# daviesthomas/cudaNeuralRender

Hardware: AMD Instinct MI355X
Metric: Mray-steps/s at 1024^2, plane_1.h5 (frames/s in config.fps) (higher is better)
Workload: dtype f32

## Files before the change

cudaneuralrender_amd/csrc/nr_mlp16.h:

```cpp
#pragma once
#include <type_traits>

#include "nr_device.h"
#include "nr_mlp16_asm.h"

#ifndef NR_MLP16_EXP
#define NR_MLP16_EXP 0
#endif

namespace nr {

typedef float f32x4 __attribute__((ext_vector_type(4)));

__device__ __forceinline__ uint32_t pl16(uint32_t a, uint32_t b, int half) {
    const auto r = __builtin_amdgcn_permlane16_swap(a, b, false, false);
    return half ? r[1] : r[0];
}
__device__ __forceinline__ uint32_t pl32(uint32_t a, uint32_t b, int half) {
    const auto r = __builtin_amdgcn_permlane32_swap(a, b, false, false);
    return half ? r[1] : r[0];
}

template <int NT>
__device__ __forceinline__ float tile_outputs(const float zt[4]) {
// ... 46 lines not shown
#pragma unroll
    for (int t = 0; t < NT; ++t)
#pragma unroll
        for (int i = 0; i < 8; ++i) a[t][i] = k[t][i];
}

template <int NT, int PART = 0, bool CL = false, int NH = 0, bool MK = false>
__device__ __forceinline__ float mlp16_fp32_nt(const float *__restrict__ s, int in0, int nh_rt, float fr, float x,
                                               float y, float z, uint32_t (*mk)[2] = nullptr) {
    const int nh = NH > 0 ? NH : nh_rt;
    auto relu = [](float v) { return CL ? __builtin_amdgcn_fmed3f(v, 0.0f, 1.0f) : fmaxf(v, 0.0f); };
    auto mark = [](uint32_t m, float act, int pos) { return (min(__float_as_uint(act), 1u) << pos) | m; };
    const int lane = lane_id(), g = lane >> 4;
    float a[NT][8];
    f32x4 c[NT][2];
    {
        const float w0 = s[PK_L0W + lane], w1 = s[PK_L0W + 64 + lane];
        uint32_t t0 = __float_as_uint(x), t1 = __float_as_uint(y), t2 = __float_as_uint(z);
        uint32_t t3 = __float_as_uint(in0 == 4 ? fr : 0.0f);
        auto r = __builtin_amdgcn_permlane32_swap(t0, t2, false, false);
        t0 = r[0]; t2 = r[1];
        r = __builtin_amdgcn_permlane32_swap(t1, t3, false, false);
        t1 = r[0]; t3 = r[1];
        r = __builtin_amdgcn_permlane16_swap(t0, t1, false, false);
        t0 = r[0]; t1 = r[1];
        r = __builtin_amdgcn_permlane16_swap(t2, t3, false, false);
        t2 = r[0]; t3 = r[1];
        const float bt[4] = {__uint_as_float(t0), __uint_as_float(t1), __uint_as_float(t2), __uint_as_float(t3)};
#pragma unroll
        for (int t = 0; t < NT; ++t) {
            c[t][0] = __builtin_amdgcn_mfma_f32_16x16x4f32(w0, bt[t], f32x4{0.0f, 0.0f, 0.0f, 0.0f}, 0, 0, 0);
            c[t][1] = __builtin_amdgcn_mfma_f32_16x16x4f32(w1, bt[t], f32x4{0.0f, 0.0f, 0.0f, 0.0f}, 0, 0, 0);
        }
        const float4 *bb = reinterpret_cast<const float4 *>(s + PK_L0B + g * 8);
        const float4 blo = bb[0], bhi = bb[1];
        const float bias[8] = {blo.x, blo.y, blo.z, blo.w, bhi.x, bhi.y, bhi.z, bhi.w};
        const float s0 = s[pk_final(nh) + 33];
#pragma unroll
        for (int t = 0; t < NT; ++t)
#pragma unroll
            for (int mt = 0; mt < 2; ++mt)
#pragma unroll
                for (int r = 0; r < 4; ++r) {
                    a[t][4 * mt + r] = relu(__builtin_fmaf(c[t][mt][r], s0, bias[4 * mt + r]));
                    if constexpr (MK) mk[t][0] = mark(mk[t][0], a[t][4 * mt + r], 4 * mt + r);
                }
    }
    constexpr bool STREAM = NT <= 2 && CL && NH == 7 && PART == 0;
    if constexpr (STREAM) f32_hidden7_stream<NT>(s, a);
    for (int jl = 0; jl < (STREAM ? 0 : nh); ++jl) {
        const float *L = s + PK_HID + jl * PK_HID_STRIDE;
        float4 wq[4];
#pragma unroll
        for (int q = 0; q < 4; ++q) wq[q] = reinterpret_cast<const float4 *>(L)[q * 64 + lane];
#pragma unroll
        for (int st = 0; st < 8; ++st) {
#pragma unroll
            for (int mt = 0; mt < 2; ++mt) {
                const int m = 2 * st + mt;
                const float4 wv = wq[m >> 2];
                const float w = (m & 3) == 0 ? wv.x : ((m & 3) == 1 ? wv.y : ((m & 3) == 2 ? wv.z : wv.w));
#pragma unroll
                for (int t = 0; t < NT; ++t)
                    c[t][mt] = __builtin_amdgcn_mfma_f32_16x16x4f32(
                        w, a[t][st], st == 0 ? f32x4{0.0f, 0.0f, 0.0f, 0.0f} : c[t][mt], 0, 0, 0);
            }
        }
        const float4 *bb = reinterpret_cast<const float4 *>(L + 1024 + g * 8);
        const float4 blo = bb[0], bhi = bb[1];
        const float bias[8] = {blo.x, blo.y, blo.z, blo.w, bhi.x, bhi.y, bhi.z, bhi.w};
#pragma unroll
        for (int t = 0; t < NT; ++t)
#pragma unroll
            for (int mt = 0; mt < 2; ++mt)
#pragma unroll
                for (int r = 0; r < 4; ++r) a[t][4 * mt + r] = relu(c[t][mt][r] + bias[4 * mt + r]);
        if constexpr (MK) {
            const int pos = 8 * ((jl + 1) & 3);
#pragma unroll
            for (int t = 0; t < NT; ++t)
#pragma unroll
                for (int k = 0; k < 8; ++k) {
                    if (jl + 1 < 4) mk[t][0] = mark(mk[t][0], a[t][k], pos + k);
                    else mk[t][1] = mark(mk[t][1], a[t][k], pos + k);
                }
        }
    }
    if constexpr (PART != 0) return a[0][0] + a[NT - 1][7];
    if constexpr (NT >= 3) {
        float b[4][8];
#pragma unroll
        for (int k = 0; k < 8; ++k) {
            uint32_t t0 = __float_as_uint(a[0][k]), t1 = __float_as_uint(a[1][k]);
            uint32_t t2 = __float_as_uint(a[2][k]), t3 = NT > 3 ? __float_as_uint(a[NT > 3 ? 3 : 0][k]) : 0u;
            auto r = __builtin_amdgcn_permlane32_swap(t0, t2, false, false);
            t0 = r[0]; t2 = r[1];
            r = __builtin_amdgcn_permlane32_swap(t1, t3, false, false);
            t1 = r[0]; t3 = r[1];
            r = __builtin_amdgcn_permlane16_swap(t0, t1, false, false);
            t0 = r[0]; t1 = r[1];
            r = __builtin_amdgcn_permlane16_swap(t2, t3, false, false);
            t2 = r[0]; t3 = r[1];
            b[0][k] = __uint_as_float(t0); b[1][k] = __uint_as_float(t1);
            b[2][k] = __uint_as_float(t2); b[3][k] = __uint_as_float(t3);
        }
        const float4 *wf4 = reinterpret_cast<const float4 *>(s + pk_final(nh));
        float acc = 0.0f;
#pragma unroll
        for (int q = 0; q < 8; ++q) {
            const float4 w = wf4[q];
            const int gg = q >> 1, k0 = 4 * (q & 1);
            acc = __builtin_fmaf(w.x, b[gg][k0 + 0], acc);
            acc = __builtin_fmaf(w.y, b[gg][k0 + 1], acc);
            acc = __builtin_fmaf(w.z, b[gg][k0 + 2], acc);
            acc = __builtin_fmaf(w.w, b[gg][k0 + 3], acc);
        }
        return acc + s[pk_final(nh) + 32];
    }
    const float *wf = s + pk_final(nh) + g * 8;
    const float bf = s[pk_final(nh) + 32];
    float w8[8];
#pragma unroll
    for (int k = 0; k < 8; ++k) w8[k] = wf[k];
    float zt[4] = {0.0f, 0.0f, 0.0f, 0.0f};
#pragma unroll
    for (int t = 0; t < NT; ++t) {
        float acc = 0.0f;
#pragma unroll
        for (int k = 0; k < 8; ++k) acc = __builtin_fmaf(w8[k], a[t][k], acc);
#pragma unroll
        for (int q = 1; q < 4; ++q) {
            float nacc = from_prev_group(acc, q);
#pragma unroll
            for (int k = 0; k < 8; ++k) nacc = __builtin_fmaf(w8[k], a[t][k], nacc);
            acc = (g == q) ? nacc : acc;
        }
        zt[t] = acc + bf;
    }
    return tile_outputs<NT>(zt);
}

__device__ __forceinline__ bool inputs_in_bound_f32(float x, float y, float z, float f) {
    const bool ok = __builtin_fabsf(x) <= F32_INPUT_BOUND && __builtin_fabsf(y) <= F32_INPUT_BOUND &&
                    __builtin_fabsf(z) <= F32_INPUT_BOUND && __builtin_fabsf(f) <= F32_INPUT_BOUND;
    return __ballot(!ok) == 0;
}

template <bool ST = false>
__device__ __forceinline__ float mlp16_fp32(const float *__restrict__ s, int in0, int nh, float fr, float x, float y,
                                            float z, uint32_t tmask, bool cl) {
    const int nt = 32 - __clz((int)tmask);
    if (cl) {
        if (nt >= 4) return mlp16_fp32_nt<4, 0, true>(s, in0, nh, fr, x, y, z);
        if (nt == 3) return mlp16_fp32_nt<3, 0, true>(s, in0, nh, fr, x, y, z);
        if (nt == 2) return mlp16_fp32_nt<2, 0, true>(s, in0, nh, fr, x, y, z);
        if (ST && NR_F32_STREAM && nh == 7) return mlp16_fp32_nt<1, 0, true, 7>(s, in0, nh, fr, x, y, z);
        if (nt == 2) return mlp16_fp32_nt<2, 0, true>(s, in0, nh, fr, x, y, z);
        return mlp16_fp32_nt<1, 0, true>(s, in0, nh, fr, x, y, z);
    }
    return mlp16_fp32_nt<4>(s, in0, nh, fr, x, y, z);
}
template <bool ST = false>
__device__ __forceinline__ float mlp16_fp32(const MlpArgs &M, const float *s, float fr, float x, float y, float z,
                                            uint32_t tmask) {
    return mlp16_fp32<ST>(s, M.in0, M.nh, fr, x, y, z, tmask, M.f32_clamp && inputs_in_bound_f32(x, y, z, fr));
}

__device__ __forceinline__ int prune_ks(unsigned long long kb, int l) { return 4 + (int)((kb >> (3 * l)) & 7ull); }

template <int NT>
__device__ __forceinline__ float mlp16_fp32_pruned_nt(const float *__restrict__ s, int in0, int nh, unsigned long long kb,
                                                      float fr, float x, float y, float z, uint32_t &flag) {
    auto relu = [](float v) { return __builtin_amdgcn_fmed3f(v, 0.0f, 1.0f); };
    const int lane = lane_id(), g = lane >> 4;
    f32x4 av[NT][2];
    f32x4 c[NT][2];
    uint32_t fl = 0;
    auto skipped = [&](int k) {
#pragma unroll
        for (int t = 0; t < NT; t += 2) fl |= __float_as_uint(av[t][k >> 2][k & 3]) | __float_as_uint(av[t + 1 < NT ? t + 1 : t][k >> 2][k & 3]);
    };
    {
        const float w0 = s[PK_L0W + lane], w1 = s[PK_L0W + 64 + lane];
        uint32_t t0 = __float_as_uint(x), t1 = __float_as_uint(y), t2 = __float_as_uint(z);
        uint32_t t3 = __float_as_uint(in0 == 4 ? fr : 0.0f);
        auto r = __builtin_amdgcn_permlane32_swap(t0, t2, false, false);
        t0 = r[0]; t2 = r[1];
        r = __builtin_amdgcn_permlane32_swap(t1, t3, false, false);
        t1 = r[0]; t3 = r[1];
        r = __builtin_amdgcn_permlane16_swap(t0, t1, false, false);
        t0 = r[0]; t1 = r[1];
        r = __builtin_amdgcn_permlane16_swap(t2, t3, false, false);
        t2 = r[0]; t3 = r[1];
        const float bt[4] = {__uint_as_float(t0), __uint_as_float(t1), __uint_as_float(t2), __uint_as_float(t3)};
#pragma unroll
        for (int t = 0; t < NT; ++t) {
            c[t][0] = __builtin_amdgcn_mfma_f32_16x16x4f32(w0, bt[t], f32x4{0.0f, 0.0f, 0.0f, 0.0f}, 0, 0, 0);
            c[t][1] = __builtin_amdgcn_mfma_f32_16x16x4f32(w1, bt[t], f32x4{0.0f, 0.0f, 0.0f, 0.0f}, 0, 0, 0);
        }
        const float4 *bb = reinterpret_cast<const float4 *>(s + PK_L0B + g * 8);
        const float4 blo = bb[0], bhi = bb[1];
        const float bias[8] = {blo.x, blo.y, blo.z, blo.w, bhi.x, bhi.y, bhi.z, bhi.w};
        const float s0 = s[pk_final(nh) + 33];
#pragma unroll
        for (int t = 0; t < NT; ++t)
#pragma unroll
            for (int mt = 0; mt < 2; ++mt)
#pragma unroll
                for (int r = 0; r < 4; ++r) av[t][mt][r] = relu(__builtin_fmaf(c[t][mt][r], s0, bias[4 * mt + r]));
    }
    for (int jl = 0; jl < nh; ++jl) {
        const int ks = prune_ks(kb, jl);
        const float *L = s + PK_HID + jl * PK_HID_STRIDE;
        float4 wq[2];
#pragma unroll
        for (int q = 0; q < 2; ++q) wq[q] = reinterpret_cast<const float4 *>(L)[q * 64 + lane];
#pragma unroll
        for (int st = 0; st < 8; ++st) {
            if (st < 4 || st < ks) {
                float2 w2 = {0.0f, 0.0f};
                if (st >= 4) w2 = reinterpret_cast<const float2 *>(L)[((st >> 1) * 64 + lane) * 2 + (st & 1)];
#pragma unroll
                for (int mt = 0; mt < 2; ++mt) {
                    const int m = 2 * st + mt;
                    const float4 wv = wq[st < 4 ? m >> 2 : 0];
                    const float w4 = (m & 3) == 0 ? wv.x : ((m & 3) == 1 ? wv.y : ((m & 3) == 2 ? wv.z : wv.w));
                    const float w = st < 4 ? w4 : (mt ? w2.y : w2.x);
#pragma unroll
                    for (int t = 0; t < NT; ++t)
                        c[t][mt] = __builtin_amdgcn_mfma_f32_16x16x4f32(
                            w, av[t][st >> 2][st & 3], st == 0 ? f32x4{0.0f, 0.0f, 0.0f, 0.0f} : c[t][mt], 0, 0, 0);
                }
            }
        }
        if (ks < 8) {
#pragma unroll
            for (int k = 4; k < 8; ++k)
                if (k >= ks) skipped(k);
        }
        const float4 *bb = reinterpret_cast<const float4 *>(L + 1024 + g * 8);
        const float4 blo = bb[0], bhi = bb[1];
        const float bias[8] = {blo.x, blo.y, blo.z, blo.w, bhi.x, bhi.y, bhi.z, bhi.w};
#pragma unroll
        for (int t = 0; t < NT; ++t)
#pragma unroll
            for (int mt = 0; mt < 2; ++mt)
#pragma unroll
                for (int r = 0; r < 4; ++r) av[t][mt][r] = relu(c[t][mt][r] + bias[4 * mt + r]);
    }
    const int ks = prune_ks(kb, nh);
    const float4 *wf4 = reinterpret_cast<const float4 *>(s + pk_final(nh));
    float acc = 0.0f;
#pragma unroll
    for (int k = 0; k < 8; ++k) {
        if (k < 4 || k < ks) {
            uint32_t t0 = __float_as_uint(av[0][k >> 2][k & 3]), t1 = NT > 1 ? __float_as_uint(av[NT > 1 ? 1 : 0][k >> 2][k & 3]) : 0u;
            uint32_t t2 = NT > 2 ? __float_as_uint(av[NT > 2 ? 2 : 0][k >> 2][k & 3]) : 0u;
            uint32_t t3 = NT > 3 ? __float_as_uint(av[NT > 3 ? 3 : 0][k >> 2][k & 3]) : 0u;
            auto r = __builtin_amdgcn_permlane32_swap(t0, t2, false, false);
            t0 = r[0]; t2 = r[1];
            r = __builtin_amdgcn_permlane32_swap(t1, t3, false, false);
            t1 = r[0]; t3 = r[1];
            r = __builtin_amdgcn_permlane16_swap(t0, t1, false, false);
            t0 = r[0]; t1 = r[1];
            r = __builtin_amdgcn_permlane16_swap(t2, t3, false, false);
            t2 = r[0]; t3 = r[1];
            const float4 w = wf4[k];
            acc = __builtin_fmaf(w.x, __uint_as_float(t0), acc);
            acc = __builtin_fmaf(w.y, __uint_as_float(t1), acc);
            acc = __builtin_fmaf(w.z, __uint_as_float(t2), acc);
            acc = __builtin_fmaf(w.w, __uint_as_float(t3), acc);
        }
    }
    if (ks < 8) {
#pragma unroll
        for (int k = 4; k < 8; ++k)
            if (k >= ks) skipped(k);
    }
    flag = fl;
    return acc + s[pk_final(nh) + 32];
}

__device__ __forceinline__ float mlp16_fp32_pruned(const MlpArgs &M, const float *s, float fr, float x, float y, float z,
                                                   uint32_t tmask, uint32_t &redo) {
    redo = 0;
    if (M.pkp) {
        if (M.f32_clamp && inputs_in_bound_f32(x, y, z, fr)) {
            const int nt = 32 - __clz((int)tmask);
            const unsigned long long kb = M.ks_bits;
            uint32_t fl = 0;
            float v;
            if (nt >= 4) v = mlp16_fp32_pruned_nt<4>(s, M.in0, M.nh, kb, fr, x, y, z, fl);
            else if (nt == 3) v = mlp16_fp32_pruned_nt<3>(s, M.in0, M.nh, kb, fr, x, y, z, fl);
            else if (nt == 2) v = mlp16_fp32_pruned_nt<2>(s, M.in0, M.nh, kb, fr, x, y, z, fl);
            else v = mlp16_fp32_pruned_nt<1>(s, M.in0, M.nh, kb, fr, x, y, z, fl);
            if (__builtin_expect(__ballot(fl != 0) == 0, 1)) return v;
            redo = 1;
        }
        return mlp16_fp32_nt<4>((const float *)(const __attribute__((address_space(1))) float *)M.pk, M.in0, M.nh, fr, x, y, z);
    }
    return mlp16_fp32_nt<4>(s, M.in0, M.nh, fr, x, y, z);
}

#ifndef NR_UNIT_GROUP
#define NR_UNIT_GROUP 8
#endif
typedef float f32x32 __attribute__((ext_vector_type(32)));
__device__ __forceinline__ constexpr int unit_reg(int u) { return 16 * ((u >> 2) & 1) + (u & 3) + 4 * (u >> 3); }

template <bool L0>
__device__ __forceinline__ void units_epilogue(const f32x32 &c, f32x32 &a, const float *bias, float s0, int h) {
    const float4 *bb = reinterpret_cast<const float4 *>(bias + 4 * h);
#pragma unroll
    for (int q = 0; q < 4; ++q) {
        const float4 b4 = bb[2 * q];
        const float b[4] = {b4.x, b4.y, b4.z, b4.w};
#pragma unroll
        for (int i = 0; i < 4; ++i) {
            const int r = 4 * q + i;
            a[r] = __builtin_amdgcn_fmed3f(L0 ? __builtin_fmaf(c[r], s0, b[i]) : c[r] + b[i], 0.0f, 1.0f);
            a[16 + r] = __builtin_amdgcn_fmed3f(L0 ? __builtin_fmaf(c[16 + r], s0, b[i]) : c[16 + r] + b[i], 0.0f, 1.0f);
        }
    }
#pragma unroll
    for (int r = 0; r < 16; ++r) {
        auto t = __builtin_amdgcn_permlane32_swap(__float_as_uint(a[r]), __float_as_uint(a[16 + r]), false, false);
        a[r] = __uint_as_float(t[0]);
        a[16 + r] = __uint_as_float(t[1]);
    }
}

__device__ __forceinline__ float mlp64_fp32_units(const float *__restrict__ s, int in0, int nh, float fr, float x, float y,
                                                  float z, unsigned long long live, uint32_t &nskip) {
    int lane = lane_id();
    asm volatile("" : "+v"(lane));
    const int row = lane & 31, h = lane >> 5;
    f32x32 a, c;
    {
        const float *w = s + PK_L0W + row;
        c = __builtin_amdgcn_mfma_f32_32x32x1f32(w[0], x, f32x32{}, 0, 0, 0);
        c = __builtin_amdgcn_mfma_f32_32x32x1f32(w[32], y, c, 0, 0, 0);
        c = __builtin_amdgcn_mfma_f32_32x32x1f32(w[64], z, c, 0, 0, 0);
        if (in0 == 4) c = __builtin_amdgcn_mfma_f32_32x32x1f32(w[96], fr, c, 0, 0, 0);
        units_epilogue<true>(c, a, s + PK_L0B, s[pk_final(nh) + 33], h);
    }
    uint32_t ni = 0;
    constexpr int UG = NR_UNIT_GROUP;
    for (int jl = 0; jl < nh; ++jl) {
        const float *L = s + PK_HID + jl * PK_HID_STRIDE;
        const float4 *W4 = reinterpret_cast<const float4 *>(L) + row;
#pragma unroll
        for (int g = 0; g < 32 / UG; ++g) {
            float w[UG];
#pragma unroll
            for (int q = 0; q < UG / 4; ++q) {
                const float4 wv = W4[(UG / 4 * g + q) * 32];
                w[4 * q] = wv.x; w[4 * q + 1] = wv.y; w[4 * q + 2] = wv.z; w[4 * q + 3] = wv.w;
            }
            unsigned long long m[UG];
#pragma unroll
            for (int i = 0; i < UG; ++i) {
                m[i] = __builtin_amdgcn_ballot_w64(__float_as_uint(a[unit_reg(UG * g + i)]) != 0u) & live;
            }
#pragma unroll
            for (int i = 0; i < UG; ++i) {
                const int u = UG * g + i;
                if (u == 0) c = __builtin_amdgcn_mfma_f32_32x32x1f32(w[i], a[unit_reg(u)], f32x32{}, 0, 0, 0);
                else if (m[i]) {
                    c = __builtin_amdgcn_mfma_f32_32x32x1f32(w[i], a[unit_reg(u)], c, 0, 0, 0);
                    ++ni;
                }
            }
        }
        units_epilogue<false>(c, a, L + 1024, 0.0f, h);
    }
    nskip += 31u * (uint32_t)nh - ni;
    const float4 *wf4 = reinterpret_cast<const float4 *>(s + pk_final(nh));
    float acc = 0.0f;
#pragma unroll
    for (int q = 0; q < 8; ++q) {
        const float4 wv = wf4[q];
        acc = __builtin_fmaf(wv.x, a[unit_reg(4 * q + 0)], acc);
        acc = __builtin_fmaf(wv.y, a[unit_reg(4 * q + 1)], acc);
        acc = __builtin_fmaf(wv.z, a[unit_reg(4 * q + 2)], acc);
        acc = __builtin_fmaf(wv.w, a[unit_reg(4 * q + 3)], acc);
    }
    return acc + s[pk_final(nh) + 32];
}

__device__ __forceinline__ float mlp64_fp32_units(const MlpArgs &M, const float *s, float fr, float x, float y, float z,
                                                  unsigned long long live, uint32_t &nskip, uint32_t &neval) {
    if (inputs_in_bound_f32(x, y, z, fr)) {
        ++neval;
        return mlp64_fp32_units(s, M.in0, M.nh, fr, x, y, z, live, nskip);
    }
    return mlp16_fp32_nt<4>((const float *)(const __attribute__((address_space(1))) float *)M.pk, M.in0, M.nh, fr, x, y, z);
}

template <int PREC> struct Lowp;
template <> struct Lowp<NR_PRECISION_BF16> { typedef __bf16 e; typedef bf16x8 v8; };
template <> struct Lowp<NR_PRECISION_FP16> { typedef _Float16 e; typedef f16x8 v8; };
typedef uint32_t u32x4 __attribute__((ext_vector_type(4)));

__device__ __forceinline__ void half_views(float v, float &v0, float &v1) {
    const auto r = __builtin_amdgcn_permlane32_swap(__float_as_uint(v), __float_as_uint(v), false, false);
    v0 = __uint_as_float(r[0]);
    v1 = __uint_as_float(r[1]);
}

template <int PREC>
__device__ __forceinline__ f32x16 mfma32(const typename Lowp<PREC>::v8 &a, const typename Lowp<PREC>::v8 &b,
                                         const f32x16 &c) {
    if constexpr (PREC == NR_PRECISION_BF16) return __builtin_amdgcn_mfma_f32_32x32x16_bf16(a, b, c, 0, 0, 0);
    else return __builtin_amdgcn_mfma_f32_32x32x16_f16(a, b, c, 0, 0, 0);
}

template <int PREC>
__device__ __forceinline__ float dot2(uint32_t a, uint32_t b, float c) {
    typedef __bf16 bf16x2 __attribute__((ext_vector_type(2)));
    typedef _Float16 f16x2 __attribute__((ext_vector_type(2)));
    if constexpr (PREC == NR_PRECISION_BF16)
        return __builtin_amdgcn_fdot2_f32_bf16(__builtin_bit_cast(bf16x2, a), __builtin_bit_cast(bf16x2, b), c, false);
    else
        return __builtin_amdgcn_fdot2(__builtin_bit_cast(f16x2, a), __builtin_bit_cast(f16x2, b), c, false);
}

template <int PREC>
__device__ __forceinline__ typename Lowp<PREC>::v8 relu_pack8(const f32x16 &c, int s) {
    typedef typename Lowp<PREC>::e e16;
    typedef e16 e16x2 __attribute__((ext_vector_type(2)));
    typedef short s16x2 __attribute__((ext_vector_type(2)));
    typedef float f32x2 __attribute__((ext_vector_type(2)));
    u32x4 w;
#pragma unroll
    for (int q = 0; q < 4; ++q) {
        const f32x2 v = {c[8 * s + 2 * q], c[8 * s + 2 * q + 1]};
        const s16x2 h = __builtin_bit_cast(s16x2, __builtin_convertvector(v, e16x2));
        w[q] = __builtin_bit_cast(uint32_t, __builtin_elementwise_max(h, (s16x2){0, 0}));
    }
    return __builtin_bit_cast(typename Lowp<PREC>::v8, w);
}

__device__ __forceinline__ f32x16 load_bias16(const float *b) {
    const float4 *q = reinterpret_cast<const float4 *>(b);
    const float4 a0 = q[0], a1 = q[1], a2 = q[2], a3 = q[3];
    return f32x16{a0.x, a0.y, a0.z, a0.w, a1.x, a1.y, a1.z, a1.w, a2.x, a2.y, a2.z, a2.w, a3.x, a3.y, a3.z, a3.w};
}

#define NR_CVC(o, a, b) "v_cvt_pk_bf16_f32 %" #o ", %" #a ", %" #b " clamp\n"
__device__ __forceinline__ void relu_clamp_bf16_x2(const f32x16 &c, const f32x16 &d, u32x4 (&k)[2][2]) {
    const uint32_t t0 = __float_as_uint(c[0]) & 1u, t1 = __float_as_uint(d[0]) & 1u;
    asm(NR_CVC(0, 16, 17) NR_CVC(1, 18, 19) NR_CVC(2, 20, 21) NR_CVC(3, 22, 23)
        NR_CVC(4, 24, 25) NR_CVC(5, 26, 27) NR_CVC(6, 28, 29) NR_CVC(7, 30, 31)
        NR_CVC(8, 32, 33) NR_CVC(9, 34, 35) NR_CVC(10, 36, 37) NR_CVC(11, 38, 39)
        NR_CVC(12, 40, 41) NR_CVC(13, 42, 43) NR_CVC(14, 44, 45) NR_CVC(15, 46, 47)
        "s_nop 1"
        : "=&v"(k[0][0][0]), "=&v"(k[0][0][1]), "=&v"(k[0][0][2]), "=&v"(k[0][0][3]),
          "=&v"(k[0][1][0]), "=&v"(k[0][1][1]), "=&v"(k[0][1][2]), "=&v"(k[0][1][3]),
          "=&v"(k[1][0][0]), "=&v"(k[1][0][1]), "=&v"(k[1][0][2]), "=&v"(k[1][0][3]),
          "=&v"(k[1][1][0]), "=&v"(k[1][1][1]), "=&v"(k[1][1][2]), "=&v"(k[1][1][3])
        : "v"(c[0]), "v"(c[1]), "v"(c[2]), "v"(c[3]), "v"(c[4]), "v"(c[5]), "v"(c[6]), "v"(c[7]),
          "v"(c[8]), "v"(c[9]), "v"(c[10]), "v"(c[11]), "v"(c[12]), "v"(c[13]), "v"(c[14]), "v"(c[15]),
          "v"(d[0]), "v"(d[1]), "v"(d[2]), "v"(d[3]), "v"(d[4]), "v"(d[5]), "v"(d[6]), "v"(d[7]),
          "v"(d[8]), "v"(d[9]), "v"(d[10]), "v"(d[11]), "v"(d[12]), "v"(d[13]), "v"(d[14]), "v"(d[15]),
          "v"(t0), "v"(t1));
}
__device__ __forceinline__ void relu_clamp_bf16_x4(const f32x16 &c0, const f32x16 &c1, const f32x16 &c2, const f32x16 &c3,
                                                   u32x4 (&k)[4][2]) {
    const uint32_t t0 = __float_as_uint(c0[0]) & 1u, t1 = __float_as_uint(c1[0]) & 1u;
    const uint32_t t2 = __float_as_uint(c2[0]) & 1u, t3 = __float_as_uint(c3[0]) & 1u;
    asm(NR_CVC(0, 32, 33) NR_CVC(1, 34, 35) NR_CVC(2, 36, 37) NR_CVC(3, 38, 39)
         NR_CVC(4, 40, 41) NR_CVC(5, 42, 43) NR_CVC(6, 44, 45) NR_CVC(7, 46, 47)
         NR_CVC(8, 48, 49) NR_CVC(9, 50, 51) NR_CVC(10, 52, 53) NR_CVC(11, 54, 55)
         NR_CVC(12, 56, 57) NR_CVC(13, 58, 59) NR_CVC(14, 60, 61) NR_CVC(15, 62, 63)
         NR_CVC(16, 64, 65) NR_CVC(17, 66, 67) NR_CVC(18, 68, 69) NR_CVC(19, 70, 71)
         NR_CVC(20, 72, 73) NR_CVC(21, 74, 75) NR_CVC(22, 76, 77) NR_CVC(23, 78, 79)
         NR_CVC(24, 80, 81) NR_CVC(25, 82, 83) NR_CVC(26, 84, 85) NR_CVC(27, 86, 87)
         NR_CVC(28, 88, 89) NR_CVC(29, 90, 91) NR_CVC(30, 92, 93) NR_CVC(31, 94, 95)
        "s_nop 1"
        : "=&v"(k[0][0][0]), "=&v"(k[0][0][1]), "=&v"(k[0][0][2]), "=&v"(k[0][0][3]),
          "=&v"(k[0][1][0]), "=&v"(k[0][1][1]), "=&v"(k[0][1][2]), "=&v"(k[0][1][3]),
          "=&v"(k[1][0][0]), "=&v"(k[1][0][1]), "=&v"(k[1][0][2]), "=&v"(k[1][0][3]),
          "=&v"(k[1][1][0]), "=&v"(k[1][1][1]), "=&v"(k[1][1][2]), "=&v"(k[1][1][3]),
          "=&v"(k[2][0][0]), "=&v"(k[2][0][1]), "=&v"(k[2][0][2]), "=&v"(k[2][0][3]),
          "=&v"(k[2][1][0]), "=&v"(k[2][1][1]), "=&v"(k[2][1][2]), "=&v"(k[2][1][3]),
          "=&v"(k[3][0][0]), "=&v"(k[3][0][1]), "=&v"(k[3][0][2]), "=&v"(k[3][0][3]),
          "=&v"(k[3][1][0]), "=&v"(k[3][1][1]), "=&v"(k[3][1][2]), "=&v"(k[3][1][3])
        : "v"(c0[0]), "v"(c0[1]), "v"(c0[2]), "v"(c0[3]), "v"(c0[4]), "v"(c0[5]), "v"(c0[6]), "v"(c0[7]),
          "v"(c0[8]), "v"(c0[9]), "v"(c0[10]), "v"(c0[11]), "v"(c0[12]), "v"(c0[13]), "v"(c0[14]), "v"(c0[15]),
          "v"(c1[0]), "v"(c1[1]), "v"(c1[2]), "v"(c1[3]), "v"(c1[4]), "v"(c1[5]), "v"(c1[6]), "v"(c1[7]),
          "v"(c1[8]), "v"(c1[9]), "v"(c1[10]), "v"(c1[11]), "v"(c1[12]), "v"(c1[13]), "v"(c1[14]), "v"(c1[15]),
          "v"(c2[0]), "v"(c2[1]), "v"(c2[2]), "v"(c2[3]), "v"(c2[4]), "v"(c2[5]), "v"(c2[6]), "v"(c2[7]),
          "v"(c2[8]), "v"(c2[9]), "v"(c2[10]), "v"(c2[11]), "v"(c2[12]), "v"(c2[13]), "v"(c2[14]), "v"(c2[15]),
          "v"(c3[0]), "v"(c3[1]), "v"(c3[2]), "v"(c3[3]), "v"(c3[4]), "v"(c3[5]), "v"(c3[6]), "v"(c3[7]),
          "v"(c3[8]), "v"(c3[9]), "v"(c3[10]), "v"(c3[11]), "v"(c3[12]), "v"(c3[13]), "v"(c3[14]), "v"(c3[15]),
          "v"(t0), "v"(t1), "v"(t2), "v"(t3));
}
__device__ __forceinline__ void relu_clamp_bf16_x1(const f32x16 &c, u32x4 (&k)[2]) {
    const uint32_t t0 = __float_as_uint(c[0]) & 1u;
    asm(NR_CVC(0, 8, 9) NR_CVC(1, 10, 11) NR_CVC(2, 12, 13) NR_CVC(3, 14, 15)
        NR_CVC(4, 16, 17) NR_CVC(5, 18, 19) NR_CVC(6, 20, 21) NR_CVC(7, 22, 23)
        "s_nop 1"
        : "=&v"(k[0][0]), "=&v"(k[0][1]), "=&v"(k[0][2]), "=&v"(k[0][3]),
          "=&v"(k[1][0]), "=&v"(k[1][1]), "=&v"(k[1][2]), "=&v"(k[1][3])
        : "v"(c[0]), "v"(c[1]), "v"(c[2]), "v"(c[3]), "v"(c[4]), "v"(c[5]), "v"(c[6]), "v"(c[7]),
          "v"(c[8]), "v"(c[9]), "v"(c[10]), "v"(c[11]), "v"(c[12]), "v"(c[13]), "v"(c[14]), "v"(c[15]),
          "v"(t0));
}
#undef NR_CVC

template <int PREC, int NT, bool CL>
__device__ __forceinline__ void relu_pack_tiles(const f32x16 (&acc)[NT], typename Lowp<PREC>::v8 (&k)[NT][2]) {
    typedef typename Lowp<PREC>::v8 v8;
    if constexpr (CL && PREC == NR_PRECISION_BF16) {
        u32x4 u[NT][2];
        if constexpr (NT == 4) relu_clamp_bf16_x4(acc[0], acc[1], acc[2], acc[3], u);
        else if constexpr (NT == 2) relu_clamp_bf16_x2(acc[0], acc[1], u);
        else relu_clamp_bf16_x1(acc[0], u[0]);
#pragma unroll
        for (int t = 0; t < NT; ++t)
#pragma unroll
            for (int s = 0; s < 2; ++s) k[t][s] = __builtin_bit_cast(v8, u[t][s]);
    } else {
#pragma unroll
        for (int t = 0; t < NT; ++t)
#pragma unroll
            for (int s = 0; s < 2; ++s) k[t][s] = relu_pack8<PREC>(acc[t], s);
    }
}

template <int PREC> struct Hidden32W {
    typename Lowp<PREC>::v8 a0, a1;
    f32x16 b;
};
template <int PREC>
__device__ __forceinline__ Hidden32W<PREC> hidden32_load(const uint16_t *__restrict__ lp, const float *__restrict__ fl,
                                                         int jl) {
    typedef typename Lowp<PREC>::v8 v8;
    const int lane = lane_id(), h = lane >> 5;
    const v8 *A = reinterpret_cast<const v8 *>(lp + LP32_HID + jl * LP32_HSTRIDE);
    return Hidden32W<PREC>{A[lane], A[64 + lane], load_bias16(fl + 32 + 32 * jl + 16 * h)};
}

template <int PREC, int NT, bool CL>
__device__ __forceinline__ void hidden32(const Hidden32W<PREC> &w, f32x16 (&acc)[NT]) {
    typedef typename Lowp<PREC>::v8 v8;
    v8 k[NT][2];
    relu_pack_tiles<PREC, NT, CL>(acc, k);
#pragma unroll
    for (int t = 0; t < NT; ++t) acc[t] = mfma32<PREC>(w.a1, k[t][1], mfma32<PREC>(w.a0, k[t][0], w.b));
}

template <int PREC, int NT, int NH, bool CL>
__device__ __forceinline__ void hidden_layers(const uint16_t *__restrict__ lp, const float *__restrict__ fl, int nh,
                                              f32x16 (&acc)[NT]) {
    if constexpr (NH > 0) {
#pragma unroll
        for (int jl = 0; jl < NH; ++jl) hidden32<PREC, NT, CL>(hidden32_load<PREC>(lp, fl, jl), acc);
    } else {
        for (int jl = 0; jl < nh; ++jl) hidden32<PREC, NT, CL>(hidden32_load<PREC>(lp, fl, jl), acc);
    }
}

template <int PREC>
__device__ __forceinline__ uint32_t cvt2(float a, float b) {
    typedef typename Lowp<PREC>::e e16;
    typedef e16 e16x2 __attribute__((ext_vector_type(2)));
    typedef float f32x2 __attribute__((ext_vector_type(2)));
    return __builtin_bit_cast(uint32_t, __builtin_convertvector((f32x2){a, b}, e16x2));
}
template <int PREC>
__device__ __forceinline__ float lo16f(uint32_t p) {
    if constexpr (PREC == NR_PRECISION_BF16) return __uint_as_float(p << 16);
    else return (float)__builtin_bit_cast(_Float16, (uint16_t)(p & 0xffffu));
}
template <int PREC>
__device__ __forceinline__ float hi16f(uint32_t p) {
    if constexpr (PREC == NR_PRECISION_BF16) return __uint_as_float(p & 0xffff0000u);
    else return (float)__builtin_bit_cast(_Float16, (uint16_t)(p >> 16));
}



template <int PREC, int NT, int NH, bool CL>
__device__ __forceinline__ float mlp32_lowp_nt(const uint16_t *__restrict__ lp, const float *__restrict__ fl, int in0,
                                               int nh_rt, float fr, float x, float y, float z) {
    typedef typename Lowp<PREC>::v8 v8;
    const int nh = NH > 0 ? NH : nh_rt;
    const int lane = lane_id(), h = lane >> 5;
    f32x16 acc[NT];
    {
        const uint32_t p0 = cvt2<PREC>(x, y);
        const float dx = x - lo16f<PREC>(p0), dy = y - hi16f<PREC>(p0);
        const uint32_t q = cvt2<PREC>(z, dx);
        const uint32_t r = cvt2<PREC>(dy, z - lo16f<PREC>(q));
        uint32_t f = 0;
        if (in0 == 4) {
            const uint32_t f0 = cvt2<PREC>(fr, 0.0f);
            f = cvt2<PREC>(fr, fr - lo16f<PREC>(f0));
        }
        const uint32_t qf = (q & 0xffffu) | (f << 16);
        const auto w0 = __builtin_amdgcn_permlane32_swap(p0, p0, false, false);
        const auto w1 = __builtin_amdgcn_permlane32_swap(q, qf, false, false);
        const auto w2 = __builtin_amdgcn_permlane32_swap(r, 0u, false, false);
        const auto w3 = __builtin_amdgcn_permlane32_swap(f, 0u, false, false);
        const v8 A = reinterpret_cast<const v8 *>(lp)[lane];
        const f32x16 b0 = load_bias16(fl + 16 * h);
#pragma unroll
        for (int t = 0; t < NT; ++t)
            acc[t] = mfma32<PREC>(A, __builtin_bit_cast(v8, (u32x4){w0[t], w1[t], w2[t], w3[t]}), b0);
    }
    hidden_layers<PREC, NT, NH, CL>(lp, fl, nh, acc);
    const u32x4 *F4 = reinterpret_cast<const u32x4 *>(lp + lp32_final(nh));
    const u32x4 wf[2] = {F4[h], F4[2 + h]};
    const float bf = fl[32 + 32 * nh];
    v8 k[NT][2];
    relu_pack_tiles<PREC, NT, CL>(acc, k);
    float zt[NT];
#pragma unroll
    for (int t = 0; t < NT; ++t) {
        float a = 0.0f;
#pragma unroll
        for (int st = 0; st < 2; ++st) {
            const u32x4 kv = __builtin_bit_cast(u32x4, k[t][st]);
#pragma unroll
            for (int q = 0; q < 4; ++q) a = dot2<PREC>(kv[q], wf[st][q], a);
        }
        zt[t] = a;
    }
    float z0, z1;
    if constexpr (NT == 1) {
        half_views(zt[0], z0, z1);
    } else {
        const auto r = __builtin_amdgcn_permlane32_swap(__float_as_uint(zt[0]), __float_as_uint(zt[1]), false, false);
        z0 = __uint_as_float(r[0]);
        z1 = __uint_as_float(r[1]);
    }
    return (z0 + z1) + bf;
}


template <int PREC, bool CL>
__device__ __forceinline__ void mlp7_x4_stream(const uint16_t *__restrict__ lp, const float *__restrict__ fl,
                                               u32x4 (&k)[4][2]) {
    typedef uint32_t u32x8 __attribute__((ext_vector_type(8)));
    const int lane = lane_id();
    const uint32_t va = lds_addr(lp) + 16u * (uint32_t)lane, vb = lds_addr(fl) + 64u * (uint32_t)(lane >> 5);
    f32x16 c0, c1, c2, c3, bb0, bb1;
    u32x8 ab0, ab1;
#define NR_STREAM_OPERANDS                                                                                          \
    : "+{v[64:67]}"(k[0][0]), "=&{v[68:71]}"(k[0][1]), "+{v[72:75]}"(k[1][0]), "=&{v[76:79]}"(k[1][1]),            \
      "+{v[80:83]}"(k[2][0]), "=&{v[84:87]}"(k[2][1]), "+{v[88:91]}"(k[3][0]), "=&{v[92:95]}"(k[3][1]),            \
      "=&{v[0:15]}"(c0), "=&{v[16:31]}"(c1), "=&{v[32:47]}"(c2), "=&{v[48:63]}"(c3), "=&{v[96:103]}"(ab0),         \
      "=&{v[104:111]}"(ab1), "=&{v[112:127]}"(bb0), "=&{v[128:143]}"(bb1)                                          \
    : [va] "v"(va), [vb] "v"(vb)                                                                                   \
    : "memory"
    if constexpr (PREC == NR_PRECISION_BF16 && CL) asm volatile(NR_HID7_BF16_CLAMP NR_STREAM_OPERANDS);
    else if constexpr (PREC == NR_PRECISION_BF16) asm volatile(NR_HID7_BF16_MAX NR_STREAM_OPERANDS);
    else asm volatile(NR_HID7_F16_MAX NR_STREAM_OPERANDS);
#undef NR_STREAM_OPERANDS
}

template <int PREC, bool CL>
__device__ __forceinline__ void mlp7_x4_stream_s16(const uint16_t *__restrict__ lp, const float *__restrict__ fl,
                                                   u32x4 (&k)[4][2]) {
    typedef uint32_t u32x8 __attribute__((ext_vector_type(8)));
    const int lane = lane_id();
    const uint32_t va = lds_addr(lp) + 16u * (uint32_t)lane, vb0 = lds_addr(fl) + 64u * (uint32_t)(lane >> 5),
                   vb = lds_addr(fl) + 32u * (uint32_t)(lane >> 4);
    f32x16 c0, c1, c2, c3;
    u32x8 ab0, ab1, bb0, bb1;
#define NR_S16_OPERANDS                                                                                             \
    : "+{v[64:67]}"(k[0][0]), "=&{v[68:71]}"(k[0][1]), "+{v[72:75]}"(k[1][0]), "=&{v[76:79]}"(k[1][1]),            \
      "+{v[80:83]}"(k[2][0]), "=&{v[84:87]}"(k[2][1]), "+{v[88:91]}"(k[3][0]), "=&{v[92:95]}"(k[3][1]),            \
      "=&{v[0:15]}"(c0), "=&{v[16:31]}"(c1), "=&{v[32:47]}"(c2), "=&{v[48:63]}"(c3), "=&{v[96:103]}"(ab0),         \
      "=&{v[104:111]}"(ab1), "=&{v[112:119]}"(bb0), "=&{v[120:127]}"(bb1)                                          \
    : [va] "v"(va), [vb0] "v"(vb0), [vb] "v"(vb)                                                                   \
// ... 397 lines not shown
```

Measured before the change: 12060.

## Software-pipeline LDS weight and bias reads in units MLP with inline asm

Replaces compiler-scheduled LDS loads of hidden-layer weights and biases with explicit ds_read_b128 inline asm, issued one group ahead and paired with manual lgkmcnt waits. Each weight quad is prefetched while the MFMAs of the previous quad run, and the next layer's first weights and biases are fetched during the epilogue. The aim is to hide LDS latency behind MFMA work. In exchange it adds volatile asm that limits compiler scheduling, blanket lgkmcnt(0) waits, and fixed assumptions about layout offsets.

```diff
diff --git a/cudaneuralrender_amd/csrc/nr_mlp16.h b/cudaneuralrender_amd/csrc/nr_mlp16.h
--- a/cudaneuralrender_amd/csrc/nr_mlp16.h
+++ b/cudaneuralrender_amd/csrc/nr_mlp16.h
@@ -372,24 +372,49 @@
     return mlp16_fp32_nt<4>(s, M.in0, M.nh, fr, x, y, z);
 }
 
-#ifndef NR_UNIT_GROUP
-#define NR_UNIT_GROUP 8
-#endif
+constexpr int UNIT_GROUP = 8;
 typedef float f32x32 __attribute__((ext_vector_type(32)));
+typedef float f32x4 __attribute__((ext_vector_type(4)));
 __device__ __forceinline__ constexpr int unit_reg(int u) { return 16 * ((u >> 2) & 1) + (u & 3) + 4 * (u >> 3); }
 
+__device__ __forceinline__ uint32_t lds_addr(const float *p) {
+    return (uint32_t)(uintptr_t)(const __attribute__((address_space(3))) float *)p;
+}
+template <int OFF>
+__device__ __forceinline__ void units_wread(uint32_t addr, f32x4 &w) {
+    asm volatile("ds_read_b128 %0, %1 offset:%2" : "=&v"(w) : "v"(addr), "n"(OFF));
+}
+template <int Q>
+__device__ __forceinline__ void units_bread(uint32_t addr, f32x4 &b0, f32x4 &b1) {
+    asm volatile("ds_read_b128 %0, %2 offset:%3\n\tds_read_b128 %1, %2 offset:%4"
+                 : "=&v"(b0), "=&v"(b1)
+                 : "v"(addr), "n"(32 * Q), "n"(32 * Q + 32));
+}
+__device__ __forceinline__ void units_wait(f32x4 &w) { asm volatile("s_waitcnt lgkmcnt(0)" : "+v"(w)); }
+__device__ __forceinline__ void units_wait(f32x4 &b0, f32x4 &b1) {
+    asm volatile("s_waitcnt lgkmcnt(0)" : "+v"(b0), "+v"(b1));
+}
+__device__ __forceinline__ void units_wait(f32x4 &w, f32x4 &b0, f32x4 &b1) {
+    asm volatile("s_waitcnt lgkmcnt(0)" : "+v"(w), "+v"(b0), "+v"(b1));
+}
+
 template <bool L0>
-__device__ __forceinline__ void units_epilogue(const f32x32 &c, f32x32 &a, const float *bias, float s0, int h) {
-    const float4 *bb = reinterpret_cast<const float4 *>(bias + 4 * h);
+__device__ __forceinline__ void units_epilogue(const f32x32 &c, f32x32 &a, f32x4 &b0, f32x4 &b1, uint32_t ba, float s0,
+                                               uint32_t wa, f32x4 &w) {
+    f32x4 b2, b3;
+    units_wait(b0, b1);
+    units_bread<2>(ba, b2, b3);
+    units_wread<0>(wa, w);
 #pragma unroll
     for (int q = 0; q < 4; ++q) {
-        const float4 b4 = bb[2 * q];
-        const float b[4] = {b4.x, b4.y, b4.z, b4.w};
+        if (q == 2) units_wait(w, b2, b3);
+        const f32x4 &bq = q == 0 ? b0 : q == 1 ? b1 : q == 2 ? b2 : b3;
 #pragma unroll
         for (int i = 0; i < 4; ++i) {
             const int r = 4 * q + i;
-            a[r] = __builtin_amdgcn_fmed3f(L0 ? __builtin_fmaf(c[r], s0, b[i]) : c[r] + b[i], 0.0f, 1.0f);
-            a[16 + r] = __builtin_amdgcn_fmed3f(L0 ? __builtin_fmaf(c[16 + r], s0, b[i]) : c[16 + r] + b[i], 0.0f, 1.0f);
+            const float b = bq[i];
+            a[r] = __builtin_amdgcn_fmed3f(L0 ? __builtin_fmaf(c[r], s0, b) : c[r] + b, 0.0f, 1.0f);
+            a[16 + r] = __builtin_amdgcn_fmed3f(L0 ? __builtin_fmaf(c[16 + r], s0, b) : c[16 + r] + b, 0.0f, 1.0f);
         }
     }
 #pragma unroll
@@ -406,43 +431,58 @@
     asm volatile("" : "+v"(lane));
     const int row = lane & 31, h = lane >> 5;
     f32x32 a, c;
+    uint32_t wa = lds_addr(s) + 4u * (nh > 0 ? PK_HID : 0) + 16u * row;
+    uint32_t ba = lds_addr(s) + 4u * PK_L0B + 16u * h;
+    f32x4 w;
     {
-        const float *w = s + PK_L0W + row;
-        c = __builtin_amdgcn_mfma_f32_32x32x1f32(w[0], x, f32x32{}, 0, 0, 0);
-        c = __builtin_amdgcn_mfma_f32_32x32x1f32(w[32], y, c, 0, 0, 0);
-        c = __builtin_amdgcn_mfma_f32_32x32x1f32(w[64], z, c, 0, 0, 0);
-        if (in0 == 4) c = __builtin_amdgcn_mfma_f32_32x32x1f32(w[96], fr, c, 0, 0, 0);
-        units_epilogue<true>(c, a, s + PK_L0B, s[pk_final(nh) + 33], h);
-    }
+        f32x4 b0, b1;
+        units_bread<0>(ba, b0, b1);
+        const float *w0 = s + PK_L0W + row;
+        c = __builtin_amdgcn_mfma_f32_32x32x1f32(w0[0], x, f32x32{}, 0, 0, 0);
+        c = __builtin_amdgcn_mfma_f32_32x32x1f32(w0[32], y, c, 0, 0, 0);
+        c = __builtin_amdgcn_mfma_f32_32x32x1f32(w0[64], z, c, 0, 0, 0);
+        if (in0 == 4) c = __builtin_amdgcn_mfma_f32_32x32x1f32(w0[96], fr, c, 0, 0, 0);
+        units_epilogue<true>(c, a, b0, b1, ba, s[pk_final(nh) + 33], wa, w);
+    }
+    ba += 4u * (PK_HID + 1024 - PK_L0B);
     uint32_t ni = 0;
-    constexpr int UG = NR_UNIT_GROUP;
+    constexpr int UG = UNIT_GROUP;
     for (int jl = 0; jl < nh; ++jl) {
-        const float *L = s + PK_HID + jl * PK_HID_STRIDE;
-        const float4 *W4 = reinterpret_cast<const float4 *>(L) + row;
-#pragma unroll
-        for (int g = 0; g < 32 / UG; ++g) {
-            float w[UG];
-#pragma unroll
-            for (int q = 0; q < UG / 4; ++q) {
-                const float4 wv = W4[(UG / 4 * g + q) * 32];
-                w[4 * q] = wv.x; w[4 * q + 1] = wv.y; w[4 * q + 2] = wv.z; w[4 * q + 3] = wv.w;
+        f32x4 b0, b1;
+        unsigned long long m[UG];
+#pragma unroll
+        for (int k = 0; k < 8; ++k) {
+            if (4 * k % UG == 0) {
+#pragma unroll
+                for (int i = 0; i < UG; ++i)
+                    m[i] = __builtin_amdgcn_ballot_w64(__float_as_uint(a[unit_reg(4 * k + i)]) != 0u) & live;
             }
-            unsigned long long m[UG];
-#pragma unroll
-            for (int i = 0; i < UG; ++i) {
-                m[i] = __builtin_amdgcn_ballot_w64(__float_as_uint(a[unit_reg(UG * g + i)]) != 0u) & live;
-            }
-#pragma unroll
-            for (int i = 0; i < UG; ++i) {
-                const int u = UG * g + i;
+            f32x4 n;
+            if (k == 0) units_wread<512>(wa, n);
+            if (k == 1) units_wread<1024>(wa, n);
+            if (k == 2) units_wread<1536>(wa, n);
+            if (k == 3) units_wread<2048>(wa, n);
+            if (k == 4) units_wread<2560>(wa, n);
+            if (k == 5) units_wread<3072>(wa, n);
+            if (k == 6) units_wread<3584>(wa, n);
+            if (k == 7) units_bread<0>(ba, b0, b1);
+#pragma unroll
+            for (int i = 0; i < 4; ++i) {
+                const int u = 4 * k + i;
                 if (u == 0) c = __builtin_amdgcn_mfma_f32_32x32x1f32(w[i], a[unit_reg(u)], f32x32{}, 0, 0, 0);
-                else if (m[i]) {
+                else if (m[u % UG]) {
                     c = __builtin_amdgcn_mfma_f32_32x32x1f32(w[i], a[unit_reg(u)], c, 0, 0, 0);
                     ++ni;
                 }
             }
-        }
-        units_epilogue<false>(c, a, L + 1024, 0.0f, h);
+            if (k < 7) {
+                units_wait(n);
+                w = n;
+            }
+        }
+        if (jl + 1 < nh) wa += 4u * PK_HID_STRIDE;
+        units_epilogue<false>(c, a, b0, b1, ba, 0.0f, wa, w);
+        ba += 4u * PK_HID_STRIDE;
     }
     nskip += 31u * (uint32_t)nh - ni;
     const float4 *wf4 = reinterpret_cast<const float4 *>(s + pk_final(nh));
```

Result: faster. 12270 (median of 6 runs) (+1.7%).
